# MathsionYang/Ransac

Measured on NVIDIA B200. Metric: hypothesis x point evaluations/s (useful, whole job); ms per robust fit in config, higher is better.
Workload: dtype f32

## Files before the change

ransac_b200/csrc/pipeline.cuh:

```cuda
#pragma once
#include "strict_math.cuh"

struct RoundArgs {
    const ProblemDesc* prob;
    const int* active;
    FitState* state;
    const float* aos;
    int est, K, S, m, mstride;
    int e5_all_roots;
    int midx_shift;
    int sampler, rng, neighbors;
    uint64_t seed;
    const int* table; unsigned table_rows;
    const unsigned* growth;
    const int* knn; const int* cell_of_point; const int* members; const int* rank_in_cell; const int* cell_start;
    unsigned* cursors;
    int* seeds;
    int* samples;
    float* models_raw;
    int* nmodels;
    int* offsets;
    float* recs;
    int* mvalid;
    uint2* items;
    unsigned* item_count;
    int* part_cnt; float* part_sum; int nchunks;
    uint2* sample_scores;
    float thr, confidence;
    unsigned max_iterations;
    const unsigned* term_tables;
    int rank, nranks;
    int sprt;
    const int* pool;
    struct SprtModelResult* sprt_res;
    int* done_out;
    unsigned before_sprt;
    int limit_remaining;
    void* const* peer_win;
    void* peer_self;
    unsigned peer_seq;
    unsigned peer_cap;
    unsigned* peer_counter;
    int* peer_error;
    unsigned long long hyp_base_p1;
};

#define USAC_PEER_HEADER_BYTES 1024
#define USAC_PEER_MAX_RANKS 64
__device__ __forceinline__ uint2* peer_data(void* win, unsigned seq, unsigned cap) {
    return reinterpret_cast<uint2*>(reinterpret_cast<char*>(win) + USAC_PEER_HEADER_BYTES) + (size_t)(seq & 1u) * cap;
}
__device__ __forceinline__ unsigned* peer_flags(void* win, unsigned seq) {
    return reinterpret_cast<unsigned*>(win) + (seq & 1u) * USAC_PEER_MAX_RANKS;
}
__device__ __forceinline__ void peer_store(const RoundArgs& a, size_t idx, uint2 v) {
    for (int r = 0; r < a.nranks; r++) peer_data(a.peer_win[r], a.peer_seq, a.peer_cap)[idx] = v;
}
__device__ __forceinline__ void peer_publish(const RoundArgs& a) {
    __threadfence_system();
    __syncthreads();
    if (threadIdx.x == 0) {
        const unsigned total = gridDim.x * gridDim.y * gridDim.z;
        if (atomicAdd(a.peer_counter, 1u) == total - 1u) {
            *a.peer_counter = 0u;
            __threadfence_system();
            for (int r = 0; r < a.nranks; r++) {
                unsigned* f = peer_flags(a.peer_win[r], a.peer_seq) + a.rank;
                asm volatile("st.release.sys.global.u32 [%0], %1;" :: "l"(f), "r"(a.peer_seq) : "memory");
            }
        }
    }
}
__device__ __forceinline__ void peer_wait(const RoundArgs& a) {
    if ((int)threadIdx.x < a.nranks) {
        const unsigned* f = peer_flags(a.peer_self, a.peer_seq) + threadIdx.x;
        unsigned long long t0 = 0, t1 = 0;
        asm volatile("mov.u64 %0, %%globaltimer;" : "=l"(t0));
        for (;;) {
            unsigned v;
            asm volatile("ld.acquire.sys.global.u32 %0, [%1];" : "=r"(v) : "l"(f) : "memory");
            if ((int)(v - a.peer_seq) >= 0) break;
            asm volatile("mov.u64 %0, %%globaltimer;" : "=l"(t1));
            if (t1 - t0 > 2000000000ull) { *a.peer_error = 1; break; }
            __nanosleep(200);
        }
    }
    __syncthreads();
}

__device__ __forceinline__ void make_record(int est, const float* model, float thr, const ProblemDesc& pd, float* rec) {
    const float u = 5.9604645e-8f;
#pragma unroll
    for (int i = 0; i < USAC_REC_STRIDE; i++) rec[i] = 0.f;
    const int w = est == USAC_EST_LINE2D ? 3 : 9;
    for (int i = 0; i < w; i++) rec[i] = model[i];
    rec[REC_THR] = thr;
    const float* f = model;
    if (est == USAC_EST_HOMOGRAPHY) {
        cv_inv3x3(model, rec + REC_HINV);
        const float* g = rec + REC_HINV;
        const float T2 = 2.f * thr;
        const float bx1 = fabsf(f[0]) * pd.mx1 + fabsf(f[1]) * pd.my1 + fabsf(f[2]);
        const float by1 = fabsf(f[3]) * pd.mx1 + fabsf(f[4]) * pd.my1 + fabsf(f[5]);
        const float bz1 = fabsf(f[6]) * pd.mx1 + fabsf(f[7]) * pd.my1 + fabsf(f[8]);
        const float bx2 = fabsf(g[0]) * pd.mx2 + fabsf(g[1]) * pd.my2 + fabsf(g[2]);
        const float by2 = fabsf(g[3]) * pd.mx2 + fabsf(g[4]) * pd.my2 + fabsf(g[5]);
        const float bz2 = fabsf(g[6]) * pd.mx2 + fabsf(g[7]) * pd.my2 + fabsf(g[8]);
        const float g8 = 8.f * u;
        const float K1 = g8 * ((bx1 + by1) + (pd.mx2 + pd.my2 + 2.1f * T2) * bz1);
        const float K2 = g8 * ((bx2 + by2) + (pd.mx1 + pd.my1 + 2.1f * T2) * bz2);
        const float c0 = g8 * (pd.mx1 + pd.my1 + pd.mx2 + pd.my2 + 4.2f * T2) + 32.f * u * T2;
        rec[REC_BAND] = 1.001f * (K1 + c0 * bz1);
        rec[REC_BAND + 1] = 1.001f * K2;
    } else if (est == USAC_EST_FUNDAMENTAL) {
        const float ba = fabsf(f[0]) * pd.mx1 + fabsf(f[1]) * pd.my1 + fabsf(f[2]);
        const float bb = fabsf(f[3]) * pd.mx1 + fabsf(f[4]) * pd.my1 + fabsf(f[5]);
        const float bc = fabsf(f[0]) * pd.mx2 + fabsf(f[3]) * pd.my2 + fabsf(f[6]);
        const float bd = fabsf(f[1]) * pd.mx2 + fabsf(f[4]) * pd.my2 + fabsf(f[7]);
        const float bn = pd.mx2 * ba + pd.my2 * bb + fabsf(f[6]) * pd.mx1 + fabsf(f[7]) * pd.my1 + fabsf(f[8]);
// ... 92 lines not shown
    const ProblemDesc pd = a.prob[pid];
    FitState& st = a.state[pid];
    const uint64_t hyp = (a.hyp_base_p1 ? (uint64_t)(a.hyp_base_p1 - 1) : (uint64_t)st.samples_drawn) + j;
    int s[8];
    const int m = a.m, n = pd.n;
    if (a.rng == USAC_RNG_TABLE && pid == 0 && hyp < a.table_rows) {
        for (int i = 0; i < m; i++) s[i] = a.table[hyp * m + i];
    } else if (a.sampler == USAC_SAMPLER_PROSAC) {
        const unsigned* g = a.growth + pd.growth_off;
        const unsigned t0 = st.prosac_t, n0 = st.prosac_n, L = st.prosac_term_len;
        auto n_before = [&](int jj) -> unsigned { return jj == 0 ? n0 : max(n0, prosac_subset(g, n, m, t0 + jj - 1)); };
        unsigned n_prev = n_before(j);
        const bool term_mode = n_prev > L;
        unsigned t_next, n_next;
        if (term_mode) {
            int lo = 0, hi = j;
            while (lo < hi) { const int mid = (lo + hi) >> 1; if (n_before(mid) > L) hi = mid; else lo = mid + 1; }
            n_prev = n_before(lo);
            philox_unique(a.seed, hyp, 2, (int)min(L + 1, (unsigned)n), m, s);
            t_next = t0 + lo; n_next = n_prev;
        } else {
            const unsigned nn = max(n0, prosac_subset(g, n, m, t0 + j));
            philox_unique(a.seed, hyp, 3, (int)nn - 1, m - 1, s);
            s[m - 1] = (int)nn - 1;
            t_next = t0 + j + 1; n_next = nn;
        }
        if (j == a.K - 1) { st.prosac_t_next = t_next; st.prosac_n_next = n_next; st.prosac_largest_next = max(st.prosac_largest, n_next); }
    } else if (a.sampler == USAC_SAMPLER_NAPSAC) {
        const int* seeds = a.seeds + (size_t)slot * a.K;
        const int p = seeds[j];
        const bool uniform_by_now = a.neighbors != USAC_NEIGH_KNN && hyp >= (uint64_t)a.cursors[pd.cursor_off + 3 * (size_t)n];
        if (p < 0 || uniform_by_now) {
            philox_unique(a.seed, hyp, 0, n, m, s);
        } else {
            unsigned c = a.cursors[pd.cursor_off + p];
            const unsigned uses = a.cursors[pd.cursor_off + n + p];
            if (uses == 2u) {
                c += ((unsigned)j > (unsigned)a.K - a.cursors[pd.cursor_off + 2 * (size_t)n + p]) ? (unsigned)(m - 1) : 0u;
            } else if (uses > 2u) {
                unsigned earlier = 0;
                int i = 0;
                for (; i + 8 <= j; i += 8) {
                    int v[8];
#pragma unroll
                    for (int u = 0; u < 8; u++) v[u] = seeds[i + u];
#pragma unroll
                    for (int u = 0; u < 8; u++) earlier += (v[u] == p);
                }
                for (; i < j; i++) earlier += (seeds[i] == p);
                c += earlier * (unsigned)(m - 1);
            }
            s[0] = p;
            if (a.neighbors == USAC_NEIGH_KNN) {
                const int* row = a.knn + pd.knn_off + (size_t)pd.knn * p;
                for (int i = 1; i < m; i++) s[i] = row[pd.knn - 1 - (int)((c + i - 1) % (unsigned)pd.knn)];
            } else {
                const int cell = a.cell_of_point[pd.grid_off + p];
                const int cs = a.cell_start[pd.cell_start_off + cell];
                const int cnt = a.cell_start[pd.cell_start_off + cell + 1] - cs - 1;
                const int rk = a.rank_in_cell[pd.grid_off + p];
                for (int i = 1; i < m; i++) {
                    const int pos = (int)((c + i - 1) % (unsigned)cnt);
                    s[i] = a.members[pd.grid_off + cs + pos + (pos >= rk ? 1 : 0)];
                }
            }
        }
    } else {
        philox_unique(a.seed, hyp, 0, n, m, s);
    }
    int* dst = a.samples + ((size_t)slot * a.K + j) * m;
    for (int i = 0; i < m; i++) dst[i] = s[i];
}

__device__ __forceinline__ unsigned samples_in_reach(const RoundArgs& a, const ProblemDesc& pd, const FitState& st) {
    unsigned reach = st.max_iters;
    if (a.term_tables && pd.term_off >= 0 && st.max_iters == a.max_iterations) reach = max(reach, a.term_tables[pd.term_off + (size_t)pd.n + 1]);
    return reach;
}
template <int EST>
__global__ void __launch_bounds__(64) solve_kernel(const RoundArgs a) {
    const int slot = blockIdx.y, j = blockIdx.x * blockDim.x + threadIdx.x;
    if (j >= a.K) return;
    int* nm = a.nmodels + (size_t)slot * a.K + j;
    if (a.nranks > 1 && (j % a.nranks) != a.rank) { *nm = 0; return; }
    const int pid = a.active[slot];
    const ProblemDesc pd = a.prob[pid];
    if (a.limit_remaining) {
        const FitState& st = a.state[pid];
        const unsigned reach = samples_in_reach(a, pd, st);
        if (reach <= st.iters || (unsigned)j >= reach - st.iters) { *nm = 0; return; }
    }
    const float* pts = a.aos + (size_t)pd.aos_off * (EST == USAC_EST_LINE2D ? 2 : 4);
    int s[8];
    const int* src = a.samples + ((size_t)slot * a.K + j) * a.m;
    for (int i = 0; i < a.m; i++) s[i] = src[i];
    float out[27];
    const int k = solve_minimal<EST>(pts, s, out);
    float* dst = a.models_raw + ((size_t)slot * a.K + j) * a.S * 9;
    for (int i = 0; i < k * 9; i++) dst[i] = out[i];
    *nm = k;
}

#define E5_WARPS_PER_CTA 4
#ifndef E5_MIN_CTAS
#define E5_MIN_CTAS 1
#endif
__global__ void __launch_bounds__(32 * E5_WARPS_PER_CTA, E5_MIN_CTAS) solve_kernel_e5_warp(const RoundArgs a) {
    __shared__ double sm[E5_WARPS_PER_CTA][E5_WARP_DOUBLES];
    const int slot = blockIdx.y, w = threadIdx.x >> 5, lane = threadIdx.x & 31;
    const int j = blockIdx.x * E5_WARPS_PER_CTA + w;
    if (j >= a.K) return;
    int* nm = a.nmodels + (size_t)slot * a.K + j;
    if (a.nranks > 1 && (j % a.nranks) != a.rank) { if (lane == 0) *nm = 0; return; }
    const int pid = a.active[slot];
    const ProblemDesc pd = a.prob[pid];
    if (a.limit_remaining) {
        const FitState& st = a.state[pid];
        const unsigned reach = samples_in_reach(a, pd, st);
        if (reach <= st.iters || (unsigned)j >= reach - st.iters) { if (lane == 0) *nm = 0; return; }
    }
    const float* pts = a.aos + (size_t)pd.aos_off * 4;
    int s[8];
    const int* src = a.samples + ((size_t)slot * a.K + j) * a.m;
    for (int i = 0; i < a.m; i++) s[i] = src[i];
    float* dst = a.models_raw + ((size_t)slot * a.K + j) * a.S * 9;
    const int k = solve_essential5_warp(pts, s, dst, sm[w], a.e5_all_roots);
    if (lane == 0) *nm = k;
}
__global__ void __launch_bounds__(32 * E5_WARPS_PER_CTA, E5_MIN_CTAS) estimate_kernel_e5_warp(const float* __restrict__ pts, const int* __restrict__ samples, int K,
                                                                                int S, int all_roots, float* __restrict__ models,
                                                                                int* __restrict__ nmodels) {
    __shared__ double sm[E5_WARPS_PER_CTA][E5_WARP_DOUBLES];
    const int w = threadIdx.x >> 5, lane = threadIdx.x & 31;
    const int j = blockIdx.x * E5_WARPS_PER_CTA + w;
    if (j >= K) return;
    int s[8];
    for (int i = 0; i < 5; i++) s[i] = samples[(size_t)j * 5 + i];
    float* dst = models + (size_t)j * S * 9;
    for (int i = lane; i < S * 9; i += 32) dst[i] = 0.f;
    __syncwarp();
    const int k = solve_essential5_warp(pts, s, dst, sm[w], all_roots);
    if (lane == 0) nmodels[j] = k;
}

template <int EST>
__global__ void __launch_bounds__(64) estimate_kernel(const float* __restrict__ pts, const int* __restrict__ samples, int K, int m, int S,
                                                     float* __restrict__ models, int* __restrict__ nmodels) {
    const int j = blockIdx.x * blockDim.x + threadIdx.x;
    if (j >= K) return;
    int s[8];
    for (int i = 0; i < m; i++) s[i] = samples[(size_t)j * m + i];
    float out[27];
    for (int i = 0; i < 27; i++) out[i] = 0.f;
    const int k = solve_minimal<EST>(pts, s, out);
    for (int i = 0; i < S * 9; i++) models[(size_t)j * S * 9 + i] = out[i];
    nmodels[j] = k;
}

__device__ __forceinline__ int block_exclusive_scan(int v, int* total, int* sm ) {
    const int lane = threadIdx.x & 31, warp = threadIdx.x >> 5, nw = (blockDim.x + 31) >> 5;
    int x = v;
#pragma unroll
    for (int o = 1; o < 32; o <<= 1) { const int y = __shfl_up_sync(0xffffffffu, x, o); if (lane >= o) x += y; }
    if (lane == 31) sm[warp] = x;
    __syncthreads();
    if (warp == 0) {
        int w = lane < nw ? sm[lane] : 0;
#pragma unroll
        for (int o = 1; o < 32; o <<= 1) { const int y = __shfl_up_sync(0xffffffffu, w, o); if (lane >= o) w += y; }
        sm[lane] = w;
    }
    __syncthreads();
    const int before = (warp > 0 ? sm[warp - 1] : 0) + x - v;
    *total = sm[nw - 1];
    __syncthreads();
    return before;
}

// ... 42 lines not shown

__global__ void reduce_kernel(const RoundArgs a) {
    const int slot = blockIdx.y, j = blockIdx.x * blockDim.x + threadIdx.x;
    if (j < a.K && !(a.nranks > 1 && (j % a.nranks) != a.rank)) {
        const int k = a.nmodels[(size_t)slot * a.K + j];
        const int off = a.offsets[(size_t)slot * a.K + j];
        int bc = -1, bi = 0;
        float bs = 0.f;
        for (int i = 0; i < k; i++) {
            int c = 0;
            float s = 0.f;
            for (int ch = 0; ch < a.nchunks; ch++) {
                const size_t o = ((size_t)slot * a.nchunks + ch) * a.mstride + off + i;
                c += a.part_cnt[o];
                s += a.part_sum[o];
            }
            if (bc < 0 || score_bigger(c, s, bc, bs)) { bc = c; bs = s; bi = i; }
        }
        if (bc < 0) { bc = 0; bs = 0.f; bi = midx_none(a); }
        const int per_rank = (a.K + a.nranks - 1) / a.nranks;
        const size_t dst = (a.nranks > 1) ? ((size_t)slot * per_rank + j / a.nranks) : ((size_t)slot * a.K + j);
        const uint2 v = make_uint2(pack_cnt_midx(a, bc, bi), __float_as_uint(bs));
        if (a.peer_win) peer_store(a, (size_t)a.rank * gridDim.y * per_rank + dst, v);
        else a.sample_scores[dst] = v;
    }
    if (a.peer_win) peer_publish(a);
}

template <int SMAX>
__global__ void __launch_bounds__(256) reduce_chunks_kernel(const RoundArgs a) {
    __shared__ int s_c[8][SMAX][32];
    __shared__ float s_s[8][SMAX][32];
    const int slot = blockIdx.y, lane = threadIdx.x & 31, warp = threadIdx.x >> 5;
    const int own = blockIdx.x * 32 + lane;
    const int j = a.nranks > 1 ? own * a.nranks + a.rank : own;
    const bool mine = j < a.K;
    const int k = mine ? a.nmodels[(size_t)slot * a.K + j] : 0;
    const int off = mine ? a.offsets[(size_t)slot * a.K + j] : 0;
    for (int i = 0; i < SMAX; i++) {
        int c = 0;
        float s = 0.f;
        if (i < k)
            for (int ch = warp; ch < a.nchunks; ch += 8) {
                const size_t o = ((size_t)slot * a.nchunks + ch) * a.mstride + off + i;
                c += a.part_cnt[o];
                s += a.part_sum[o];
            }
        s_c[warp][i][lane] = c;
        s_s[warp][i][lane] = s;
    }
    __syncthreads();
    if (warp == 0 && mine) {
        int bc = -1, bi = 0;
        float bs = 0.f;
        for (int i = 0; i < k; i++) {
            int c = 0;
            float s = 0.f;
            for (int w = 0; w < 8; w++) { c += s_c[w][i][lane]; s += s_s[w][i][lane]; }
            if (bc < 0 || score_bigger(c, s, bc, bs)) { bc = c; bs = s; bi = i; }
        }
        if (bc < 0) { bc = 0; bs = 0.f; bi = midx_none(a); }
        const int per_rank = (a.K + a.nranks - 1) / a.nranks;
        const size_t dst = (a.nranks > 1) ? ((size_t)slot * per_rank + own) : ((size_t)slot * a.K + j);
        const uint2 v = make_uint2(pack_cnt_midx(a, bc, bi), __float_as_uint(bs));
        if (a.peer_win) peer_store(a, (size_t)a.rank * gridDim.y * per_rank + dst, v);
        else a.sample_scores[dst] = v;
    }
    if (a.peer_win) peer_publish(a);
}

struct SelKey { unsigned long long key; int j; };
__device__ __forceinline__ SelKey sel_max(SelKey a, SelKey b) { return (b.key > a.key) ? b : a; }

__global__ void __launch_bounds__(256) select_kernel(const RoundArgs a, const uint2* __restrict__ scores_all) {
    __shared__ unsigned long long s_key[8];
    __shared__ int s_j[8];
    __shared__ int s_stop[8];
    __shared__ int s_T;
    __shared__ unsigned s_useful;
    const int slot = blockIdx.x;
    const int pid = a.active[slot];
    FitState& st = a.state[pid];
    if (a.peer_win) peer_wait(a);
    if (st.done) return;
    const ProblemDesc pd = a.prob[pid];
    const unsigned* table = a.term_tables + pd.term_off;
    const int K = a.K, R = a.nranks;
    const int per_rank = (K + R - 1) / R;
    const uint2* sc = scores_all;
    const bool peer = a.peer_win != nullptr;
    if (peer) sc = peer_data(a.peer_self, a.peer_seq, a.peer_cap);
    auto load = [&](int j) -> uint2 {
        if (peer) return __ldcv(sc + ((size_t)(j % R) * gridDim.x + slot) * per_rank + j / R);
        return (R > 1) ? sc[((size_t)(j % R) * gridDim.x + slot) * per_rank + j / R] : sc[(size_t)slot * K + j];
    };
    const unsigned long long carry_key = score_key(st.best_cnt, st.best_sum);
    const unsigned iters0 = st.iters, carry_max = st.max_iters;
    const int none = midx_none(a);

    const int per = (K + blockDim.x - 1) / blockDim.x;
    const int j0 = threadIdx.x * per, j1 = min(j0 + per, K);
    SelKey mine = {0ull, -1};
    for (int j = j0; j < j1; j++) {
        const uint2 v = load(j);
        if (packed_midx(a, v.x) == none) continue;
        SelKey c = {score_key(packed_cnt(a, v.x), __uint_as_float(v.y)), j};
        mine = sel_max(mine, c);
    }
    const int lane = threadIdx.x & 31, warp = threadIdx.x >> 5;
    SelKey inc = mine;
#pragma unroll
    for (int o = 1; o < 32; o <<= 1) {
        const SelKey left = {__shfl_up_sync(0xffffffffu, inc.key, o), __shfl_up_sync(0xffffffffu, inc.j, o)};
        if (lane >= o) inc = sel_max(left, inc);
    }
    if (lane == 31) { s_key[warp] = inc.key; s_j[warp] = inc.j; }
    __syncthreads();
    SelKey run = {carry_key, -1};
    for (int w = 0; w < warp; w++) { const SelKey c = {s_key[w], s_j[w]}; run = sel_max(run, c); }
    {
        const SelKey excl = {__shfl_up_sync(0xffffffffu, inc.key, 1), __shfl_up_sync(0xffffffffu, inc.j, 1)};
        if (lane > 0) run = sel_max(run, excl);
    }
    int stop = K;
    SelKey at_stop = run;
    for (int j = j0; j < j1; j++) {
        const uint2 v = load(j);
        if (packed_midx(a, v.x) != none) { SelKey c = {score_key(packed_cnt(a, v.x), __uint_as_float(v.y)), j}; run = sel_max(run, c); }
        const unsigned mi = (run.j < 0) ? carry_max : table[(unsigned)(run.key >> 32)];
        if (iters0 + (unsigned)j + 1u >= mi) { stop = j; at_stop = run; break; }
    }
    {
        int wmin = stop;
#pragma unroll
        for (int o = 16; o; o >>= 1) wmin = min(wmin, __shfl_xor_sync(0xffffffffu, wmin, o));
        if (lane == 0) s_stop[warp] = wmin;
    }
    __syncthreads();
    if (threadIdx.x == 0) {
        int T = K;
        for (int t = 0; t < (int)(blockDim.x >> 5); t++) T = min(T, s_stop[t]);
        s_T = T;
        s_useful = 0;
    }
    __syncthreads();
    const int T = s_T;
    {
        unsigned u = 0;
        const int* nmod = a.nmodels + (size_t)slot * K;
        for (int j = j0; j < j1 && j <= T; j++) u += (unsigned)nmod[j];
        if (u) atomicAdd(&s_useful, u);
    }
    __syncthreads();
    const bool owner = (T < K) ? (stop == T) : (threadIdx.x == blockDim.x - 1);
    if (owner) {
        const SelKey best = (T < K) ? at_stop : run;
        if (best.j >= 0) {
            const uint2 v = load(best.j);
            st.best_cnt = packed_cnt(a, v.x);
            st.best_sum = __uint_as_float(v.y);
            st.best_hyp = (long long)st.samples_drawn + best.j;
            st.best_midx = packed_midx(a, v.x);
            st.max_iters = table[(unsigned)st.best_cnt];
        }
        st.iters = iters0 + (unsigned)min(T + 1, K);
        st.done = (T < K) || !(st.iters < st.max_iters);
        st.samples_drawn += (unsigned)K;
        st.rounds += 1;
        st.round_pending = 1;
        st.useful_evals += (unsigned long long)s_useful * (unsigned long long)pd.n;
    }
}

template <int EST>
__global__ void winner_kernel(const RoundArgs a, int slots) {
    const int slot = blockIdx.x * blockDim.x + threadIdx.x;
    if (slot >= slots) return;
    const int pid = a.active[slot];
    FitState& st = a.state[pid];
    if (!st.round_pending) { if (a.done_out) a.done_out[slot] = st.done; return; }
    st.round_pending = 0;
    const ProblemDesc pd = a.prob[pid];
    const long long first = (long long)st.samples_drawn - a.K;
    if (st.best_hyp >= first) {
        const int j = (int)(st.best_hyp - first);
        const int w = EST == USAC_EST_LINE2D ? 3 : 9;
        if (a.nranks == 1 || (j % a.nranks) == a.rank) {
            const float* src = a.models_raw + (((size_t)slot * a.K + j) * a.S + st.best_midx) * 9;
            for (int i = 0; i < w; i++) st.best_model[i] = src[i];
        } else {
            int s[8];
            const int* src = a.samples + ((size_t)slot * a.K + j) * a.m;
            for (int i = 0; i < a.m; i++) s[i] = src[i];
            float out[EST == USAC_EST_ESSENTIAL ? 9 * USAC_E5_MAX_ROOTS : 27];
            const float* pts = a.aos + (size_t)pd.aos_off * (EST == USAC_EST_LINE2D ? 2 : 4);
            const int k = solve_minimal<EST>(pts, s, out, a.e5_all_roots);
            if (st.best_midx < k) for (int i = 0; i < w; i++) st.best_model[i] = out[9 * st.best_midx + i];
        }
    }
    if (a.done_out) a.done_out[slot] = st.done;
    st.evals += (unsigned long long)a.mvalid[slot] * (unsigned long long)pd.n;
    st.prosac_t = st.prosac_t_next; st.prosac_n = st.prosac_n_next; st.prosac_largest = st.prosac_largest_next;
}
```

ransac_b200/csrc/usac_gpu.cu:

```cuda
#include <dlfcn.h>

#include <cub/device/device_radix_sort.cuh>
#include <cub/device/device_scan.cuh>

#include <algorithm>
#include <chrono>
#include <cmath>
#include <cstdio>
#include <cstdlib>
#include <cstring>
#include <map>
#include <string>
#include <thread>
#include <tuple>
#include <vector>

#include "essential.cuh"
#include "pipeline.cuh"
#include "score.cuh"
#include "score_sq.cuh"
#include "sprt.cuh"
#include "refit.cuh"
#include "lo.cuh"
#include "knn.cuh"
// ... 1690 lines not shown
                        if (r.good) { if (r.tested_inl > hs.best_cnt) last_improving = r.tested_inl; }
                        else { rej_inl += (unsigned long long)r.tested_inl; rej_pts += (unsigned long long)r.tested_pts; }
                        if (!r.good && hs.iters >= before_sprt) { hs.iters++; continue; }
                        inl = r.full_inl; score = (float)inl;
                    } else {
                        inl = h_scores[q].x; memcpy(&score, &h_scores[q].y, 4);
                    }
                    if (inl > hs.best_cnt || (inl == hs.best_cnt && score > hs.best_sum)) {
                        float cand[9] = {0};
                        for (int k = 0; k < w; k++) cand[k] = h_models[(size_t)q * 9 + k];
                        if (cfg->lo) {
                            const auto t0 = now();
                            rc = lo.get_model_score(cand, inl, score);
                            if (rc) return rc;
                            t_lo_round += us(t0, now()); n_lo++;
                        }
                        hs.best_cnt = inl; hs.best_sum = score; hs.best_hyp = (long long)(hyp0 + j); hs.best_midx = i;
                        for (int k = 0; k < w; k++) hs.best_model[k] = cand[k];
                        if (is_prosac) {
                            const auto t0 = now();
                            rc = fetch_mask(c, p, hs.best_model, cfg->threshold, mask, ids);
                            if (rc) return rc;
                            hs.max_iters = pterm.update(hs.iters, mask, dev_state.prosac_largest_next);
                            t_mask_round += us(t0, now()); n_mask++;
                        } else {
                            hs.max_iters = standard_termination_value((unsigned)inl, n, m, log_1_p, cfg->max_iterations);
                        }
                        if (is_sprt) hs.max_iters = std::min(hs.max_iters, sprt.upper_bound(inl));
                    }
                }
                if (!stopped) hs.iters++;
            }
            if (is_sprt) {
                const SprtTestH t = sprt.current();
                double eps = t.epsilon, delta = t.delta;
                bool redesign = false;
                if (last_improving >= 0) { eps = (float)last_improving / n; redesign = true; }
                if (rej_pts > 0) {
                    const float delta_estimated = (float)rej_inl / (unsigned)rej_pts;
                    if (delta_estimated > 0 && std::fabs(t.delta - delta_estimated) / t.delta > 0.05) { delta = delta_estimated; redesign = true; }
                }
                if (redesign) sprt.push(eps, delta, (int)iters_round_start);
                sprt.cursor = (unsigned)(((unsigned long long)sprt.cursor + 32ull * (unsigned long long)KS) % n);
                hs.sprt_ntests = (int)sprt.hist.size();
            }
            hs.prosac_t = dev_state.prosac_t_next; hs.prosac_n = dev_state.prosac_n_next; hs.prosac_largest = dev_state.prosac_largest_next;
            hs.prosac_t_next = hs.prosac_t; hs.prosac_n_next = hs.prosac_n; hs.prosac_largest_next = hs.prosac_largest;
            hs.samples_drawn += (unsigned)K;
            hs.rounds++;
            hs.evals += evals;
            hs.useful_evals += useful;
            t_lo += t_lo_round; t_mask += t_mask_round;
            t_replay += us(t_r2, now()) - t_lo_round - t_mask_round;
        }
        hs.done = 1;
        if (overlap && prelaunched > (block_round - 1) / G) CUDA_TRY(c, cudaStreamSynchronize(c->stream2));
        usac_fit_result& r = results[p];
        memset(&r, 0, sizeof(r));
        for (int i = 0; i < w; i++) r.model[i] = hs.best_model[i];
        r.inliers = hs.best_cnt; r.score = hs.best_sum; r.iterations = hs.iters; r.samples_drawn = hs.samples_drawn;
        r.best_hyp = hs.best_hyp; r.best_model_idx = hs.best_midx; r.rounds = hs.rounds; r.evals = hs.evals; r.useful_evals = hs.useful_evals;
        if (cfg->lo) { r.lo_inner_iters = lo.inner_done; r.lo_iterative_iters = lo.iterative_done; n_waves += lo.wave_count; }
        r.msac = is_sprt ? nanf("") : usac_msac_cost(pd.n, r.inliers, r.score, cfg->threshold);
    }
#undef RK
    if (trace_kernels) print_marks(c);
    if (trace)
        fprintf(stderr, "usac_gpu_fit[replay] P=%d K=%d rounds=%d: tables %.0f us, enqueue %.0f us, wait %.0f us, replay %.0f us, LO %.0f us (%d calls), "
                "PROSAC mask+update %.0f us (%d); LO waves %llu\n", P, K, n_rounds, t_tables, t_enqueue, t_wait, t_replay, t_lo, n_lo, t_mask, n_mask, n_waves);
    return USAC_OK;
}

__global__ void copy_states_kernel(const FitState* __restrict__ src, FitState* __restrict__ dst, int P) {
    const size_t words = (size_t)P * (sizeof(FitState) / 4);
    const unsigned* s = reinterpret_cast<const unsigned*>(src);
    unsigned* d = reinterpret_cast<unsigned*>(dst);
    for (size_t i = blockIdx.x * (size_t)blockDim.x + threadIdx.x; i < words; i += (size_t)gridDim.x * blockDim.x) d[i] = s[i];
}
__global__ void iota_kernel(int* __restrict__ out, int n) {
    const int i = blockIdx.x * blockDim.x + threadIdx.x;
    if (i < n) out[i] = i;
}
__global__ void __launch_bounds__(1024) compact_active_kernel(const int* __restrict__ active, const int* __restrict__ done, int slots,
                                                              int* __restrict__ next) {
    __shared__ int sm[33];
    __shared__ int base;
    if (threadIdx.x == 0) base = 0;
    __syncthreads();
    for (int q0 = 0; q0 < slots; q0 += blockDim.x) {
        const int q = q0 + threadIdx.x;
        const int keep = (q < slots && !done[q]) ? 1 : 0;
        int total;
        const int off = block_exclusive_scan(keep, &total, sm);
        if (keep) next[base + off] = active[q];
        __syncthreads();
        if (threadIdx.x == 0) base += total;
        __syncthreads();
    }
}

extern "C" int usac_gpu_fit(usac_gpu_ctx* c, const usac_fit_cfg* cfg, usac_fit_result* results) {
    if (!c || !cfg || !results) return fail(c, USAC_ERR_ARG, "fit: bad arguments");
    if (c->P <= 0) return fail(c, USAC_ERR_STATE, "fit: no points uploaded");
    if (!(cfg->threshold > 0.f) || cfg->max_iterations == 0) return fail(c, USAC_ERR_ARG, "fit: threshold and max_iterations must be positive");
    const int nranks = std::max(cfg->nranks, 1), rank = cfg->rank;
    if (rank < 0 || rank >= nranks) return fail(c, USAC_ERR_ARG, "fit: rank out of range");
    const bool peers_ready = c->peer_nranks == nranks && c->peer_rank == rank && c->peer_self;
    if (nranks > 1 && !c->allgather && !peers_ready)
        return fail(c, USAC_ERR_STATE, "fit: nranks > 1 needs usac_gpu_peer_attach, usac_gpu_nccl_init or usac_gpu_set_allgather");
    if (const char* why = check_sampler_cfg(cfg->sampler)) return fail(c, USAC_ERR_ARG, why);
    if (cfg->sampler.rng == USAC_RNG_TABLE && (!cfg->sample_table || cfg->sample_table_rows == 0)) return fail(c, USAC_ERR_ARG, "fit: empty sample table");
    if (cfg->lo != 0 && cfg->lo != 1 && cfg->lo != 2) return fail(c, USAC_ERR_ARG, "fit: lo must be 0 (none), 1 (InItLORsc) or 2 (InItFLORsc); GC / IRLS are not built");
    if (cfg->lo && c->est == USAC_EST_LINE2D) return fail(c, USAC_ERR_ARG, "fit: local optimisation of line models is not built");
    if (cfg->essential_roots != USAC_E5_ROOTS_FIRST_VALID && cfg->essential_roots != USAC_E5_ROOTS_ALL_VALID)
        return fail(c, USAC_ERR_ARG, "fit: essential_roots must be USAC_E5_ROOTS_FIRST_VALID or USAC_E5_ROOTS_ALL_VALID");
    if (cfg->essential_roots && c->est != USAC_EST_ESSENTIAL) return fail(c, USAC_ERR_ARG, "fit: essential_roots applies to essential fits only");
    if (cfg->lo && cfg->lo_sample_size && (cfg->lo_sample_size < (unsigned)usac_sample_size(c->est) + 1 || cfg->lo_sample_size > 16))
        return fail(c, USAC_ERR_ARG, "fit: lo_sample_size must lie in [sample size + 1, 16]");
    const bool host_replay = cfg->sprt || cfg->lo || cfg->sampler.sampler == USAC_SAMPLER_PROSAC;
    if (host_replay && nranks > 1) return fail(c, USAC_ERR_ARG, "fit: SPRT / PROSAC termination with hypothesis sharding is not supported");
    cudaSetDevice(c->device);
    static const bool trace = getenv("USAC_GPU_TRACE") != nullptr;
    static const bool trace_kernels = trace && atoi(getenv("USAC_GPU_TRACE")) >= 2;
    c->marks_used = 0;
#define TK(name) do { if (trace_kernels) c->mark(name); } while (0)
    auto now = [] { return std::chrono::steady_clock::now(); };
    auto us = [](std::chrono::steady_clock::time_point a, std::chrono::steady_clock::time_point b) {
        return std::chrono::duration<double, std::micro>(b - a).count(); };
    const auto t_begin = now();
    double t_enqueue = 0, t_wait = 0;
    int n_rounds = 0;
    const int P = c->P, m = usac_sample_size(c->est), S = fit_models_per_sample(c->est, cfg);
    int max_n = 0;
    for (int p = 0; p < P; p++) max_n = std::max(max_n, c->h_prob[p].n);
    if (S > 3 && max_n >= (1 << 28)) return fail(c, USAC_ERR_ARG, "fit: USAC_E5_ROOTS_ALL_VALID needs fewer than 2^28 points per problem");
    if (cfg->sprt) for (int p = 0; p < P; p++) if (!c->h_pool_set[p]) return fail(c, USAC_ERR_STATE, "fit: SPRT needs usac_gpu_set_sprt_pool for every problem");

    int K = cfg->round_size;
    if (K <= 0) K = max_n >= 100000 ? 2048 : 512;
    K = (int)std::min<unsigned>((unsigned)K, std::max(cfg->max_iterations, 1u));
    if (nranks > 1) K = ((K + nranks - 1) / nranks) * nranks;

    {
        std::vector<long long> sig = {(long long)m, (long long)__builtin_bit_cast(unsigned, cfg->confidence), (long long)cfg->max_iterations};
        for (int p = 0; p < P; p++) sig.push_back(c->h_prob[p].n);
        bool offsets_set = true;
        for (int p = 0; p < P; p++) offsets_set = offsets_set && c->h_prob[p].term_off >= 0;
        if (sig != c->term_signature || !offsets_set) {
            std::map<int, long long> by_n;
            std::vector<unsigned> all;
            if (c->term_cache.size() > 64) c->term_cache.clear();
            for (int p = 0; p < P; p++) {
                const int n = c->h_prob[p].n;
                auto it = by_n.find(n);
                if (it == by_n.end()) {
                    auto key = std::make_tuple(n, m, cfg->confidence, cfg->max_iterations);
                    auto ct = c->term_cache.find(key);
                    if (ct == c->term_cache.end()) {
                        std::vector<unsigned> t;
                        standard_termination_table((unsigned)n, m, cfg->confidence, cfg->max_iterations, t);
                        ct = c->term_cache.emplace(key, std::move(t)).first;
                    }
                    it = by_n.insert({n, (long long)all.size()}).first;
                    all.insert(all.end(), ct->second.begin(), ct->second.end());
                }
                c->h_prob[p].term_off = it->second;
            }
            CUDA_TRY(c, c->d_term.ensure(all.size()));
            CUDA_TRY(c, cudaMemcpyAsync(c->d_term.p, all.data(), sizeof(unsigned) * all.size(), cudaMemcpyHostToDevice, c->stream));
            CUDA_TRY(c, cudaStreamSynchronize(c->stream));
            c->term_signature = sig;
        }
    }
    int rc = setup_sampler_side(c, cfg->sampler);
    if (rc) return rc;
    rc = push_desc(c);
    if (rc) return rc;
    if (cfg->sampler.rng == USAC_RNG_TABLE) {
        const int n0 = c->h_prob[0].n;
        for (size_t i = 0; i < (size_t)cfg->sample_table_rows * m; i++)
            if (cfg->sample_table[i] < 0 || cfg->sample_table[i] >= n0) return fail(c, USAC_ERR_ARG, "fit: sample table index out of range");
        CUDA_TRY(c, c->d_table.ensure((size_t)cfg->sample_table_rows * m));
        CUDA_TRY(c, cudaMemcpyAsync(c->d_table.p, cfg->sample_table, sizeof(int) * (size_t)cfg->sample_table_rows * m, cudaMemcpyHostToDevice, c->stream));
    }
    if (host_replay) {
        c->score_events_used = 0; c->last_launches = 0; c->last_score_launches = 0;
        cudaEventRecord(c->ev0, c->stream);
        static const bool batch_off = getenv("USAC_GPU_SPRT_BATCH") && atoi(getenv("USAC_GPU_SPRT_BATCH")) == 0;
        const bool batch = !batch_off && c->P > 1 && cfg->sprt && !cfg->lo && cfg->sampler.sampler != USAC_SAMPLER_PROSAC && cfg->sampler.rng != USAC_RNG_TABLE;
        rc = batch ? fit_sprt_batch(c, cfg, results, K) : fit_host_replay(c, cfg, results, K);
        cudaEventRecord(c->ev1, c->stream);
        CUDA_TRY(c, cudaStreamSynchronize(c->stream));
        collect_timing(c);
        return rc;
    }
    {
        std::vector<long long> sig = {(long long)c->est, (long long)cfg->max_iterations, (long long)P};
        for (int p = 0; p < P; p++) sig.push_back(c->h_prob[p].n);
        if (sig != c->state_init_sig) {
            for (int p = 0; p < P; p++) init_state(c->h_state[p], c->h_prob[p], c->est, cfg->max_iterations, 0);
            CUDA_TRY(c, cudaMemcpyAsync(c->d_state_init.p, c->h_state, sizeof(FitState) * P, cudaMemcpyHostToDevice, c->stream));
            CUDA_TRY(c, cudaStreamSynchronize(c->stream));
            c->state_init_sig = sig;
        }
        copy_states_kernel<<<std::min(4 * c->prop.multiProcessorCount, (P * (int)(sizeof(FitState) / 4) + 255) / 256), 256, 0, c->stream>>>(
            c->d_state_init.p, c->d_state.p, P);
    }

    std::vector<int> active(P);
    for (int p = 0; p < P; p++) active[p] = p;
    int* act_cur = c->d_active.p;
    int* act_next = c->d_active2.p;
    iota_kernel<<<(P + 255) / 256, 256, 0, c->stream>>>(act_cur, P);
    int setup_launches = 2;
    c->score_events_used = 0; c->last_launches = setup_launches; c->last_score_launches = 0;
    cudaEventRecord(c->ev0, c->stream);

    const char* growth_env = getenv("USAC_GPU_ROUND_GROWTH");
    const int growth_cap = growth_env ? atoi(growth_env) : 8;
    const bool k_free = growth_cap > 1 && !cfg->sprt && cfg->sampler.sampler != USAC_SAMPLER_PROSAC && cfg->sampler.rng != USAC_RNG_TABLE;
    const int K0 = K;
    const auto t_setup = now();
    while (!active.empty()) {
        const auto t_r0 = now();
        const int slots = (int)active.size();
        if (k_free && slots < P) {
            long long kr = std::min<long long>({2048LL, (long long)P * K0 / slots, (long long)K0 * growth_cap});
            kr = std::min<long long>(kr, std::max(cfg->max_iterations, 1u));
            kr = std::max<long long>(K0, kr / 128 * 128);
            if (nranks > 1) kr = (kr + nranks - 1) / nranks * nranks;
            K = (int)kr;
        }
        int max_pairs = 0;
        for (int p : active) max_pairs = std::max(max_pairs, c->h_prob[p].n_pairs);
        const int mblocks = (K * S + USAC_SCORE_THREADS - 1) / USAC_SCORE_THREADS;
        int chunk_pairs, nchunks;
        const int expect_models = (c->est == USAC_EST_FUNDAMENTAL || c->est == USAC_EST_ESSENTIAL) ? (K + 1) / 2 : K;
        plan_chunks(c, slots, std::max(1, ((expect_models + USAC_SCORE_THREADS - 1) / USAC_SCORE_THREADS) / nranks), max_pairs, &chunk_pairs, &nchunks);
        rc = ensure_round_buffers(c, slots, K, nchunks, nranks, S);
        if (rc) return rc;
        RoundArgs a;
        fill_round_args(c, a, cfg->sampler, K, S);
        a.active = act_cur;
        a.thr = cfg->threshold; a.confidence = cfg->confidence; a.max_iterations = cfg->max_iterations;
        a.table_rows = cfg->sample_table_rows; a.rank = rank; a.nranks = nranks; a.nchunks = nchunks;
        a.sprt = cfg->sprt; a.pool = c->d_pool.p; a.sprt_res = c->d_sprt_res.p; a.done_out = c->d_done.p;
        a.limit_remaining = 1;
        a.items = c->d_items.p; a.item_count = c->d_item_count.p;
        const bool use_peer = nranks > 1 && peers_ready && (size_t)nranks * slots * ((K + nranks - 1) / nranks) <= c->peer_cap;
        if (nranks > 1 && !use_peer && !c->allgather) return fail(c, USAC_ERR_STATE, "fit: the round does not fit the peer windows and no all-gather hook is installed");
        if (use_peer) {
            a.peer_win = c->d_peer_win.p; a.peer_self = c->peer_self; a.peer_cap = c->peer_cap;
            a.peer_counter = c->d_peer_counter.p; a.peer_error = c->d_peer_error.p;
        }
        int rounds_ahead = 1;
        if (P == 1 && max_n >= 65536) rounds_ahead = (int)std::min<unsigned>(8u, (cfg->max_iterations + (unsigned)K - 1) / (unsigned)K);
        for (int ahead = 0; ahead < rounds_ahead; ahead++) {
            TK("round");
            CUDA_TRY(c, cudaMemsetAsync(c->d_item_count.p, 0, 2 * sizeof(unsigned), c->stream));

            launch_sampler(c, a, slots);
            TK("sampler");
            switch (c->est) {
                case USAC_EST_LINE2D: launch_round_est<USAC_EST_LINE2D>(c, a, slots, cfg->sprt); break;
                case USAC_EST_HOMOGRAPHY: launch_round_est<USAC_EST_HOMOGRAPHY>(c, a, slots, cfg->sprt); break;
                case USAC_EST_FUNDAMENTAL: launch_round_est<USAC_EST_FUNDAMENTAL>(c, a, slots, cfg->sprt); break;
                default: launch_round_est<USAC_EST_ESSENTIAL>(c, a, slots, cfg->sprt); break;
            }
            TK("solve");
            prepare_kernel<<<slots, (slots == 1 && K >= 1024) ? 1024 : 256, 0, c->stream>>>(a);
            c->last_launches++;
            {
                ScoreArgs sa{};
                sa.pairs = c->d_pairs.p; sa.aos = c->d_aos.p; sa.prob = c->d_prob.p; sa.active = act_cur; sa.recs = c->d_recs.p;
                sa.mvalid = c->d_mvalid.p; sa.M = K * S; sa.mstride = K * S; sa.chunk_pairs = chunk_pairs; sa.nchunks = nchunks;
                sa.part_cnt = c->d_part_cnt.p; sa.part_sum = c->d_part_sum.p;
                sa.items = c->d_items.p; sa.item_count = c->d_item_count.p;
                TK("prepare");
                launch_score(c, sa, slots, mblocks);
                TK("score");
                dim3 gr((K + 127) / 128, slots);
                if (use_peer) { a.peer_seq = ++c->peer_seq; c->peer_rounds++; }
                const dim3 grc_grid(((K + nranks - 1) / nranks + 31) / 32, slots);
                if (nchunks > 8 && S > 3) reduce_chunks_kernel<USAC_E5_MAX_ROOTS><<<grc_grid, 256, 0, c->stream>>>(a);
                else if (nchunks > 8) reduce_chunks_kernel<USAC_MAX_MODELS_PER_SAMPLE><<<grc_grid, 256, 0, c->stream>>>(a);
                else reduce_kernel<<<gr, 128, 0, c->stream>>>(a);
                c->last_launches++;
                const uint2* scores = c->d_scores.p;
                TK("reduce");
                if (nranks > 1 && !use_peer) {
                    const size_t bytes = (size_t)slots * (K / nranks) * sizeof(uint2);
                    int grc = c->allgather(c->allgather_user, c->d_scores.p, c->d_scores_all.p, bytes, (void*)c->stream);
                    if (grc) return fail(c, USAC_ERR_NCCL, "fit: all-gather failed");
                    scores = c->d_scores_all.p;
                }
                TK("allgather");
                select_kernel<<<slots, 256, 0, c->stream>>>(a, scores);
                c->last_launches++;
            }
            switch (c->est) {
                case USAC_EST_LINE2D: launch_winner_est<USAC_EST_LINE2D>(c, a, slots); break;
                case USAC_EST_HOMOGRAPHY: launch_winner_est<USAC_EST_HOMOGRAPHY>(c, a, slots); break;
                case USAC_EST_FUNDAMENTAL: launch_winner_est<USAC_EST_FUNDAMENTAL>(c, a, slots); break;
                default: launch_winner_est<USAC_EST_ESSENTIAL>(c, a, slots); break;
            }
            TK("select+winner");
        }
        compact_active_kernel<<<1, 1024, 0, c->stream>>>(act_cur, c->d_done.p, slots, act_next);
        c->last_launches++;
        std::swap(act_cur, act_next);
        CUDA_TRY(c, cudaMemcpyAsync(c->h_done, c->d_done.p, sizeof(int) * slots, cudaMemcpyDeviceToHost, c->stream));
        if (P == 1) {
            CUDA_TRY(c, cudaMemcpyAsync(c->h_state, c->d_state.p, sizeof(FitState), cudaMemcpyDeviceToHost, c->stream));
            cudaEventRecord(c->ev1, c->stream);
        }
        if (use_peer) CUDA_TRY(c, cudaMemcpyAsync(c->h_peer_error, c->d_peer_error.p, sizeof(int), cudaMemcpyDeviceToHost, c->stream));
        const auto t_r1 = now();
        CUDA_TRY(c, cudaStreamSynchronize(c->stream));
        CUDA_TRY(c, cudaGetLastError());
        if (use_peer && *c->h_peer_error) {
            cudaMemsetAsync(c->d_peer_error.p, 0, sizeof(int), c->stream);
            return fail(c, USAC_ERR_NCCL, "fit: a rank did not publish its scores within 2 s (peer exchange)");
        }
        t_enqueue += us(t_r0, t_r1); t_wait += us(t_r1, now()); n_rounds++;
        std::vector<int> next;
        for (int q = 0; q < slots; q++) if (!c->h_done[q]) next.push_back(active[q]);
        active.swap(next);
    }
    if (P != 1) {
        CUDA_TRY(c, cudaMemcpyAsync(c->h_state, c->d_state.p, sizeof(FitState) * P, cudaMemcpyDeviceToHost, c->stream));
        cudaEventRecord(c->ev1, c->stream);
        CUDA_TRY(c, cudaStreamSynchronize(c->stream));
    }
    collect_timing(c);
    const int w = c->est == USAC_EST_LINE2D ? 3 : 9;
    for (int p = 0; p < P; p++) {
        const FitState& s = c->h_state[p];
        usac_fit_result& r = results[p];
        memset(&r, 0, sizeof(r));
        for (int i = 0; i < w; i++) r.model[i] = s.best_model[i];
        r.inliers = s.best_cnt; r.score = s.best_sum; r.iterations = s.iters; r.samples_drawn = s.samples_drawn;
        r.best_hyp = s.best_hyp; r.best_model_idx = s.best_midx; r.rounds = s.rounds; r.evals = s.evals;
        r.useful_evals = s.useful_evals;
        r.msac = usac_msac_cost(c->h_prob[p].n, r.inliers, r.score, cfg->threshold);
    }
    if (trace_kernels) print_marks(c);
    if (trace)
        fprintf(stderr, "usac_gpu_fit trace: %d problems, %d rounds: setup %.0f us, enqueue %.0f us, wait %.0f us, total %.0f us (GPU events: %.0f us, scoring %.0f us)\n",
                P, n_rounds, us(t_begin, t_setup), t_enqueue, t_wait, us(t_begin, now()), c->last_total_ms * 1e3, c->last_score_ms * 1e3);
    return USAC_OK;
}

static int peer_make_window(usac_gpu_ctx* c) {
    if (c->peer_self) return USAC_OK;
    cudaSetDevice(c->device);
    const unsigned cap = 1u << 17;
    const size_t bytes = USAC_PEER_HEADER_BYTES + 2ull * cap * sizeof(uint2);
    CUDA_TRY(c, cudaMalloc(&c->peer_self, bytes));
    CUDA_TRY(c, cudaMemset(c->peer_self, 0, bytes));
    CUDA_TRY(c, c->d_peer_counter.ensure(1));
    CUDA_TRY(c, c->d_peer_error.ensure(1));
    CUDA_TRY(c, cudaMemset(c->d_peer_counter.p, 0, sizeof(unsigned)));
    CUDA_TRY(c, cudaMemset(c->d_peer_error.p, 0, sizeof(int)));
    if (!c->h_peer_error) CUDA_TRY(c, cudaMallocHost(&c->h_peer_error, sizeof(int)));
    *c->h_peer_error = 0;
    c->peer_cap = cap;
    return USAC_OK;
}

extern "C" int usac_gpu_peer_export(usac_gpu_ctx* c, char handle_out[USAC_PEER_HANDLE_BYTES]) {
    if (!c || !handle_out) return fail(c, USAC_ERR_ARG, "peer_export: bad arguments");
    static_assert(sizeof(cudaIpcMemHandle_t) == USAC_PEER_HANDLE_BYTES, "USAC_PEER_HANDLE_BYTES is the size of a CUDA IPC handle");
    int rc = peer_make_window(c);
    if (rc) return rc;
    cudaIpcMemHandle_t h;
    CUDA_TRY(c, cudaIpcGetMemHandle(&h, c->peer_self));
    memcpy(handle_out, &h, sizeof(h));
    return USAC_OK;
}

extern "C" int usac_gpu_peer_window(usac_gpu_ctx* c, void** window_out) {
    if (!c || !window_out) return fail(c, USAC_ERR_ARG, "peer_window: bad arguments");
    int rc = peer_make_window(c);
    if (rc) return rc;
    *window_out = c->peer_self;
    return USAC_OK;
}

static int peer_finish_attach(usac_gpu_ctx* c, const std::vector<void*>& wins, int rank, int nranks) {
    CUDA_TRY(c, c->d_peer_win.ensure((size_t)nranks));
    CUDA_TRY(c, cudaMemcpy(c->d_peer_win.p, wins.data(), sizeof(void*) * nranks, cudaMemcpyHostToDevice));
    c->peer_rank = rank; c->peer_nranks = nranks;
    return USAC_OK;
}

extern "C" int usac_gpu_peer_attach(usac_gpu_ctx* c, const char* handles, int rank, int nranks) {
    if (!c || !handles || rank < 0 || rank >= nranks || nranks > USAC_PEER_MAX_RANKS) return fail(c, USAC_ERR_ARG, "peer_attach: bad arguments");
    if (c->peer_nranks) return fail(c, USAC_ERR_STATE, "peer_attach: windows are already attached");
    int rc = peer_make_window(c);
// ... 131 lines not shown
```

Baseline: 1097 billion.

## Fuse sampling into solve, winner into select, and item-count reset into compact

For uniform Philox sampling on non-essential estimators, the solve kernel now draws its own minimal sample, so the separate sampler launch is skipped. On single-rank runs, select_kernel copies the winning model, writes done flags, updates evals and PROSAC state, which makes the winner kernel launch unnecessary. The item-count memset is folded into compact_active_kernel for the first round after a compaction. The goal is fewer kernel launches per round, at the cost of more work inside the select owner thread and more coupled state updates.

```diff
diff --git a/ransac_b200/csrc/pipeline.cuh b/ransac_b200/csrc/pipeline.cuh
--- a/ransac_b200/csrc/pipeline.cuh
+++ b/ransac_b200/csrc/pipeline.cuh
@@ -35,6 +35,7 @@
     struct SprtModelResult* sprt_res;
     int* done_out;
     unsigned before_sprt;
+    int sample_in_solve;
     int limit_remaining;
     void* const* peer_win;
     void* peer_self;
@@ -293,6 +294,14 @@
     const int slot = blockIdx.y, j = blockIdx.x * blockDim.x + threadIdx.x;
     if (j >= a.K) return;
     int* nm = a.nmodels + (size_t)slot * a.K + j;
+    int s[8];
+    int* smp = a.samples + ((size_t)slot * a.K + j) * a.m;
+    if (a.sample_in_solve) {
+        const int pid = a.active[slot];
+        const uint64_t hyp = (a.hyp_base_p1 ? (uint64_t)(a.hyp_base_p1 - 1) : (uint64_t)a.state[pid].samples_drawn) + j;
+        philox_unique(a.seed, hyp, 0, a.prob[pid].n, a.m, s);
+        for (int i = 0; i < a.m; i++) smp[i] = s[i];
+    }
     if (a.nranks > 1 && (j % a.nranks) != a.rank) { *nm = 0; return; }
     const int pid = a.active[slot];
     const ProblemDesc pd = a.prob[pid];
@@ -302,9 +311,8 @@
         if (reach <= st.iters || (unsigned)j >= reach - st.iters) { *nm = 0; return; }
     }
     const float* pts = a.aos + (size_t)pd.aos_off * (EST == USAC_EST_LINE2D ? 2 : 4);
-    int s[8];
-    const int* src = a.samples + ((size_t)slot * a.K + j) * a.m;
-    for (int i = 0; i < a.m; i++) s[i] = src[i];
+    if (!a.sample_in_solve)
+        for (int i = 0; i < a.m; i++) s[i] = smp[i];
     float out[27];
     const int k = solve_minimal<EST>(pts, s, out);
     float* dst = a.models_raw + ((size_t)slot * a.K + j) * a.S * 9;
@@ -513,7 +521,10 @@
     const int pid = a.active[slot];
     FitState& st = a.state[pid];
     if (a.peer_win) peer_wait(a);
-    if (st.done) return;
+    if (st.done) {
+        if (a.nranks == 1 && a.done_out && threadIdx.x == 0) a.done_out[slot] = 1;
+        return;
+    }
     const ProblemDesc pd = a.prob[pid];
     const unsigned* table = a.term_tables + pd.term_off;
     const int K = a.K, R = a.nranks;
@@ -598,8 +609,19 @@
         st.done = (T < K) || !(st.iters < st.max_iters);
         st.samples_drawn += (unsigned)K;
         st.rounds += 1;
-        st.round_pending = 1;
         st.useful_evals += (unsigned long long)s_useful * (unsigned long long)pd.n;
+        if (R == 1) {
+            if (best.j >= 0) {
+                const float* src = a.models_raw + (((size_t)slot * K + best.j) * a.S + st.best_midx) * 9;
+                const int w = a.est == USAC_EST_LINE2D ? 3 : 9;
+                for (int i = 0; i < w; i++) st.best_model[i] = src[i];
+            }
+            if (a.done_out) a.done_out[slot] = st.done;
+            st.evals += (unsigned long long)a.mvalid[slot] * (unsigned long long)pd.n;
+            st.prosac_t = st.prosac_t_next; st.prosac_n = st.prosac_n_next; st.prosac_largest = st.prosac_largest_next;
+        } else {
+            st.round_pending = 1;
+        }
     }
 }
 
diff --git a/ransac_b200/csrc/usac_gpu.cu b/ransac_b200/csrc/usac_gpu.cu
--- a/ransac_b200/csrc/usac_gpu.cu
+++ b/ransac_b200/csrc/usac_gpu.cu
@@ -1796,10 +1796,10 @@
     if (i < n) out[i] = i;
 }
 __global__ void __launch_bounds__(1024) compact_active_kernel(const int* __restrict__ active, const int* __restrict__ done, int slots,
-                                                              int* __restrict__ next) {
+                                                              int* __restrict__ next, unsigned* __restrict__ item_count) {
     __shared__ int sm[33];
     __shared__ int base;
-    if (threadIdx.x == 0) base = 0;
+    if (threadIdx.x == 0) { base = 0; item_count[0] = 0u; item_count[1] = 0u; }
     __syncthreads();
     for (int q0 = 0; q0 < slots; q0 += blockDim.x) {
         const int q = q0 + threadIdx.x;
@@ -1960,6 +1960,7 @@
         a.table_rows = cfg->sample_table_rows; a.rank = rank; a.nranks = nranks; a.nchunks = nchunks;
         a.sprt = cfg->sprt; a.pool = c->d_pool.p; a.sprt_res = c->d_sprt_res.p; a.done_out = c->d_done.p;
         a.limit_remaining = 1;
+        a.sample_in_solve = cfg->sampler.sampler == USAC_SAMPLER_UNIFORM && cfg->sampler.rng == USAC_RNG_PHILOX && c->est != USAC_EST_ESSENTIAL;
         a.items = c->d_items.p; a.item_count = c->d_item_count.p;
         const bool use_peer = nranks > 1 && peers_ready && (size_t)nranks * slots * ((K + nranks - 1) / nranks) <= c->peer_cap;
         if (nranks > 1 && !use_peer && !c->allgather) return fail(c, USAC_ERR_STATE, "fit: the round does not fit the peer windows and no all-gather hook is installed");
@@ -1971,9 +1972,10 @@
         if (P == 1 && max_n >= 65536) rounds_ahead = (int)std::min<unsigned>(8u, (cfg->max_iterations + (unsigned)K - 1) / (unsigned)K);
         for (int ahead = 0; ahead < rounds_ahead; ahead++) {
             TK("round");
-            CUDA_TRY(c, cudaMemsetAsync(c->d_item_count.p, 0, 2 * sizeof(unsigned), c->stream));
-
-            launch_sampler(c, a, slots);
+            if (n_rounds == 0 || ahead > 0)
+                CUDA_TRY(c, cudaMemsetAsync(c->d_item_count.p, 0, 2 * sizeof(unsigned), c->stream));
+
+            if (!a.sample_in_solve) launch_sampler(c, a, slots);
             TK("sampler");
             switch (c->est) {
                 case USAC_EST_LINE2D: launch_round_est<USAC_EST_LINE2D>(c, a, slots, cfg->sprt); break;
@@ -2012,16 +2014,19 @@
                 select_kernel<<<slots, 256, 0, c->stream>>>(a, scores);
                 c->last_launches++;
             }
-            switch (c->est) {
-                case USAC_EST_LINE2D: launch_winner_est<USAC_EST_LINE2D>(c, a, slots); break;
-                case USAC_EST_HOMOGRAPHY: launch_winner_est<USAC_EST_HOMOGRAPHY>(c, a, slots); break;
-                case USAC_EST_FUNDAMENTAL: launch_winner_est<USAC_EST_FUNDAMENTAL>(c, a, slots); break;
-                default: launch_winner_est<USAC_EST_ESSENTIAL>(c, a, slots); break;
+            if (nranks > 1) {
+                switch (c->est) {
+                    case USAC_EST_LINE2D: launch_winner_est<USAC_EST_LINE2D>(c, a, slots); break;
+                    case USAC_EST_HOMOGRAPHY: launch_winner_est<USAC_EST_HOMOGRAPHY>(c, a, slots); break;
+                    case USAC_EST_FUNDAMENTAL: launch_winner_est<USAC_EST_FUNDAMENTAL>(c, a, slots); break;
+                    default: launch_winner_est<USAC_EST_ESSENTIAL>(c, a, slots); break;
+                }
             }
             TK("select+winner");
         }
-        compact_active_kernel<<<1, 1024, 0, c->stream>>>(act_cur, c->d_done.p, slots, act_next);
+        compact_active_kernel<<<1, 1024, 0, c->stream>>>(act_cur, c->d_done.p, slots, act_next, c->d_item_count.p);
         c->last_launches++;
+        TK("compact");
         std::swap(act_cur, act_next);
         CUDA_TRY(c, cudaMemcpyAsync(c->h_done, c->d_done.p, sizeof(int) * slots, cudaMemcpyDeviceToHost, c->stream));
         if (P == 1) {
@@ -2029,6 +2034,7 @@
             cudaEventRecord(c->ev1, c->stream);
         }
         if (use_peer) CUDA_TRY(c, cudaMemcpyAsync(c->h_peer_error, c->d_peer_error.p, sizeof(int), cudaMemcpyDeviceToHost, c->stream));
+        TK("flags");
         const auto t_r1 = now();
         CUDA_TRY(c, cudaStreamSynchronize(c->stream));
         CUDA_TRY(c, cudaGetLastError());
```

After: 1104 billion (median of 6 runs). Within noise of the previous version (+0.6%).
